# ZhuorenLi/MPC_motion_planning

Measured on AMD Instinct MI355X. Metric: mpc_solves_per_sec, higher is better.
Workload: dtype f64

## Files before the change

mpc_motion_planning_amd/csrc/mpcb_api.hip:

```cpp
#include <hip/hip_runtime.h>
#include <rccl/rccl.h>
#include <dlfcn.h>

#include <cmath>
#include <cstdarg>
#include <cstdio>
#include <cstring>
#include <limits>
#include <map>
#include <mutex>
#include <string>
#include <thread>
#include <vector>

#include "mpcb_kernel_dyn.h"
#include "mpcb_dispatch.h"
#include "mpcb_eval.h"
#include "mpcb_multi.h"
#include "mpcb_plant.h"

#ifndef MPCB_WAVES_PER_SIMD
#define MPCB_WAVES_PER_SIMD 1
#endif

namespace {

constexpr double INF = std::numeric_limits<double>::infinity();
thread_local std::string g_create_error;

template <int NOBS, bool GEN, bool RK4> constexpr bool mpcb_kin_fuses = mpcbd::fuses(NOBS, GEN, RK4);
template <int NOBS> constexpr bool mpcb_dyn_fuses = mpcbd::fuses(NOBS, false, false);
__host__ __device__ inline bool mpcb_second_kind1(const mpcb_config& c, const void* z0) {
  return c.init_rollout && (c.second_start == 1 || (c.second_start == 3 && !z0));
}
__device__ __forceinline__ bool mpcb_second_attempt_here(const MpcbKArgs& a, int b, int pass) {
  if (pass != MPCB_PASS_FIRST || !mpcb_second_kind1(a.cfg, a.z0) || !a.status) return false;
  __builtin_amdgcn_fence(__ATOMIC_SEQ_CST, "workgroup");
  const int st = __builtin_nontemporal_load(a.status + (size_t)b * a.st_stride);
  return st != MPCB_ST_SOLVED && st != MPCB_ST_ACCEPTABLE && st != MPCB_ST_INFEASIBLE_X0;
}

template <int NOBS, bool GEN, bool RK4> constexpr bool mpcb_kin_restores = mpcbd::restores_here(MPCB_MODEL_KIN, NOBS, GEN, RK4);
__device__ __forceinline__ bool mpcb_resto_here(const MpcbKArgs& a, int b) {
  const MpcbKArgs& al = *wv::late_args(a);
  if (!al.resto_here || !al.status) return false;
  __builtin_amdgcn_fence(__ATOMIC_SEQ_CST, "workgroup");
  return __builtin_nontemporal_load(al.status + (size_t)b * al.st_stride) == MPCB_ST_NEEDS_RESTO;
}

template <int NOBS, bool GEN = false, bool RK4 = false>
__global__ __launch_bounds__(64, MPCB_WAVES_PER_SIMD) void mpcb_kernel_kin(const MpcbKArgs a) {
  extern __shared__ __attribute__((aligned(16))) double mpcb_lds[];
  if constexpr (mpcb_kin_fuses<NOBS, GEN, RK4>) {
    int pass = a.pass;
#pragma clang loop unroll(disable)
    for (;;) {
      mpcb_solve_kin<NOBS, GEN, false, RK4>(a, (int)blockIdx.x, mpcb_lds, pass);
      if (!mpcb_second_attempt_here(a, (int)blockIdx.x, pass)) break;
      pass = MPCB_PASS_SECOND;
    }
  } else {
    mpcb_solve_kin<NOBS, GEN, false, RK4>(a, (int)blockIdx.x, mpcb_lds, a.pass);
  }
  if constexpr (mpcb_kin_restores<NOBS, GEN, RK4>) {
    if (mpcb_resto_here(a, (int)blockIdx.x)) mpcb_solve_kin<NOBS, GEN, true, RK4>(a, (int)blockIdx.x, mpcb_lds, MPCB_PASS_RESTO);
  }
}

template <int NOBS, bool GEN = false, bool RK4 = false>
__global__ __launch_bounds__(64, 1) void mpcb_kernel_kin_resto(const MpcbKArgs a) {
  extern __shared__ __attribute__((aligned(16))) double mpcb_lds[];
  mpcb_solve_kin<NOBS, GEN, true, RK4>(a, (int)blockIdx.x, mpcb_lds, MPCB_PASS_RESTO);
}

template <int NOBS, bool GEN = false, bool RK4 = false>
__global__ __launch_bounds__(64, MPCB_WAVES_PER_SIMD) void mpcb_track_kin(const MpcbKArgs a) {
  extern __shared__ __attribute__((aligned(16))) double mpcb_lds[];
  if constexpr (mpcb_kin_fuses<NOBS, GEN, RK4>) {
    int pass = a.pass;
#pragma clang loop unroll(disable)
    for (;;) {
      mpcb_solve_kin<NOBS, GEN, false, RK4, true>(a, (int)blockIdx.x, mpcb_lds, pass);
      if (!mpcb_second_attempt_here(a, (int)blockIdx.x, pass)) break;
      pass = MPCB_PASS_SECOND;
    }
  } else {
    mpcb_solve_kin<NOBS, GEN, false, RK4, true>(a, (int)blockIdx.x, mpcb_lds, a.pass);
  }
  if constexpr (mpcb_kin_restores<NOBS, GEN, RK4>) {
    if (mpcb_resto_here(a, (int)blockIdx.x)) mpcb_solve_kin<NOBS, GEN, true, RK4, true>(a, (int)blockIdx.x, mpcb_lds, MPCB_PASS_RESTO);
  }
}

template <int NOBS, bool GEN = false, bool RK4 = false>
__global__ __launch_bounds__(64, 1) void mpcb_track_kin_resto(const MpcbKArgs a) {
  extern __shared__ __attribute__((aligned(16))) double mpcb_lds[];
  mpcb_solve_kin<NOBS, GEN, true, RK4, true>(a, (int)blockIdx.x, mpcb_lds, MPCB_PASS_RESTO);
}

template <int NOBS>
__global__ __launch_bounds__(64, MPCB_WAVES_PER_SIMD) void mpcb_kernel_dyn(const MpcbKArgs a) {
  extern __shared__ __attribute__((aligned(16))) double mpcb_lds[];
  if constexpr (mpcb_dyn_fuses<NOBS>) {
    int pass = a.pass;
#pragma clang loop unroll(disable)
    for (;;) {
      mpcb_solve_dyn<NOBS>(a, (int)blockIdx.x, mpcb_lds, pass);
      if (!mpcb_second_attempt_here(a, (int)blockIdx.x, pass)) break;
      pass = MPCB_PASS_SECOND;
    }
  } else {
    mpcb_solve_dyn<NOBS>(a, (int)blockIdx.x, mpcb_lds, a.pass);
  }
}

template <int NOBS>
__global__ __launch_bounds__(64, 1) void mpcb_kernel_dyn_resto(const MpcbKArgs a) {
  extern __shared__ __attribute__((aligned(16))) double mpcb_lds[];
  mpcb_solve_dyn<NOBS, true>(a, (int)blockIdx.x, mpcb_lds, MPCB_PASS_RESTO);
}

template <int NOBS>
__global__ __launch_bounds__(64, MPCB_WAVES_PER_SIMD) void mpcb_param_kin(const MpcbKArgs a) {
  extern __shared__ __attribute__((aligned(16))) double mpcb_lds[];
  if constexpr (mpcb_kin_fuses<NOBS, false, false>) {
    int pass = a.pass;
#pragma clang loop unroll(disable)
    for (;;) {
      mpcb_solve_kin<NOBS, false, false, false, false, true>(a, (int)blockIdx.x, mpcb_lds, pass);
      if (!mpcb_second_attempt_here(a, (int)blockIdx.x, pass)) break;
      pass = MPCB_PASS_SECOND;
    }
  } else {
    mpcb_solve_kin<NOBS, false, false, false, false, true>(a, (int)blockIdx.x, mpcb_lds, a.pass);
  }
  if constexpr (mpcb_kin_restores<NOBS, false, false>) {
    if (mpcb_resto_here(a, (int)blockIdx.x)) mpcb_solve_kin<NOBS, false, true, false, false, true>(a, (int)blockIdx.x, mpcb_lds, MPCB_PASS_RESTO);
  }
}

template <int NOBS>
__global__ __launch_bounds__(64, 1) void mpcb_param_kin_resto(const MpcbKArgs a) {
  extern __shared__ __attribute__((aligned(16))) double mpcb_lds[];
  mpcb_solve_kin<NOBS, false, true, false, false, true>(a, (int)blockIdx.x, mpcb_lds, MPCB_PASS_RESTO);
}

template <int NOBS>
__global__ __launch_bounds__(64, MPCB_WAVES_PER_SIMD) void mpcb_param_dyn(const MpcbKArgs a) {
  extern __shared__ __attribute__((aligned(16))) double mpcb_lds[];
  if constexpr (mpcb_dyn_fuses<NOBS>) {
    int pass = a.pass;
#pragma clang loop unroll(disable)
    for (;;) {
      mpcb_solve_dyn<NOBS, false, true>(a, (int)blockIdx.x, mpcb_lds, pass);
      if (!mpcb_second_attempt_here(a, (int)blockIdx.x, pass)) break;
      pass = MPCB_PASS_SECOND;
    }
  } else {
    mpcb_solve_dyn<NOBS, false, true>(a, (int)blockIdx.x, mpcb_lds, a.pass);
  }
}

template <int NOBS>
__global__ __launch_bounds__(64, 1) void mpcb_param_dyn_resto(const MpcbKArgs a) {
  extern __shared__ __attribute__((aligned(16))) double mpcb_lds[];
  mpcb_solve_dyn<NOBS, true, true>(a, (int)blockIdx.x, mpcb_lds, MPCB_PASS_RESTO);
}

template <int NX, bool PARAMS>
__global__ __launch_bounds__(64) void mpcb_eval(const MpcbEvalArgs a) {
  extern __shared__ __attribute__((aligned(16))) double mpcb_lds[];
  ::mpcb_eval<NX, PARAMS>(a, (int)blockIdx.x, mpcb_lds);
}

__global__ __launch_bounds__(64) void mpcb_multi_expand(const MpcbMultiArgs a) { mpcbm::expand(a, (int)blockIdx.x); }
__global__ __launch_bounds__(64) void mpcb_multi_select(const MpcbMultiArgs a) { mpcbm::select(a, (int)blockIdx.x); }


template <int NX>
__global__ __launch_bounds__(128) void mpcb_advance(const mpcb_config c0, const mpcb_config* __restrict__ cfgs, int B, int nz,
                                                    const double* __restrict__ z, double* __restrict__ x0, double* __restrict__ z0,
                                                    double* __restrict__ obs, double* __restrict__ x_hist, double* __restrict__ u_hist,
                                                    const int32_t* __restrict__ status, int st_stride, int step, int steps,
                                                    int move_obs, int hold, double T) {
  const int b = blockIdx.x * blockDim.x + threadIdx.x;
  if (b >= B) return;
  const mpcb_config& c = cfgs ? cfgs[b] : c0;
  double* xb = x0 + (size_t)b * NX;
  double u[2];
  mpcbp::commit<NX>(c0.N, hold, status[(size_t)b * st_stride], z + (size_t)b * nz, z0 + (size_t)b * nz, u);
  mpcbp::plant<NX>(c, T, u, move_obs, xb, obs + (size_t)b * c0.n_obs * 6);
  if (u_hist) { u_hist[((size_t)b * steps + step) * 2] = u[0]; u_hist[((size_t)b * steps + step) * 2 + 1] = u[1]; }
  if (x_hist) {
    double* h = x_hist + ((size_t)b * (steps + 1) + step + 1) * NX;
#pragma unroll
    for (int q = 0; q < NX; ++q) h[q] = xb[q];
  }
}

// ... 168 lines not shown
struct mpcb_params {
  mpcb_handle* owner = nullptr;
  int32_t B = 0;
  mpcb_config base;
  mpcb_config* d_cfgs = nullptr;
};

struct mpcb_loop {
  mpcb_handle* owner = nullptr;
  int32_t B = 0, flags = 0;
  int id = 0;
  const mpcb_params* params = nullptr;
  double* d_w = nullptr;
  double* d_z = nullptr;
  double* d_traj = nullptr;
  int32_t* d_st = nullptr;
  int32_t* d_it = nullptr;
  int32_t* d_cnt = nullptr;
};

struct mpcb_handle {
  mpcb_config cfg;
  int device = 0;
  hipStream_t stream = nullptr;
  hipStream_t first_stream = nullptr;
  std::string err;
  int nx = 4, nz = 0, ng = 0;
  void* d_buf = nullptr; size_t d_cap = 0;
  void* d_multi = nullptr; size_t multi_cap = 0;
  static constexpr int EV_RING = 256;
  std::vector<std::pair<hipEvent_t, hipEvent_t>> ev;
  int ev_head = 0, ev_pending = 0;
  int launches = 0; double total_ms = 0, last_ms = 0;
  struct Lane { hipStream_t stream = nullptr; double* d_work = nullptr; int32_t* d_st_own = nullptr; int work_cap = 0; hipEvent_t done = nullptr; bool busy = false; };
  std::vector<Lane> lanes;
  int lane_base = 0;
  int inflight() const { return lanes.empty() ? 1 : (int)lanes.size() - lane_base; }
  int next_lane = 0;
  int last_solve_lane = 0;
  hipEvent_t ev_fork = nullptr;
  std::vector<std::vector<hipEvent_t>> marks;
  std::vector<double> tgrid_host;
  ncclComm_t comm = nullptr; int world = 1, rank = 0;
  std::vector<mpcb_handle*> peers;
  double* d_gather = nullptr; size_t gather_cap = 0;
  double* d_red = nullptr;
  double* d_tgrid = nullptr; double T0 = 0;
  hipEvent_t ev_sync = nullptr;
  size_t gathered_rows = 0;
  int64_t gathered_B = 0;
  std::vector<mpcb_params*> params;
  std::vector<mpcb_loop*> loops;
  int loops_created = 0;
  bool resto_in_launch = true;
  bool lane0_own_stream = true;
  bool skip_empty_pass = true;
};

namespace {

int fail(mpcb_handle* h, int code, const char* fmt, ...) {
  char buf[512];
  va_list ap; va_start(ap, fmt); vsnprintf(buf, sizeof buf, fmt, ap); va_end(ap);
  if (h) h->err = buf; else g_create_error = buf;
  return code;
}
#define HIP_TRY(h, expr)                                                                         \
  do { hipError_t e_ = (expr); if (e_ != hipSuccess) return fail(h, MPCB_E_DEVICE, "%s: %s", #expr, hipGetErrorString(e_)); } while (0)

struct Rccl {
  decltype(&ncclGetUniqueId) GetUniqueId; decltype(&ncclCommInitRank) CommInitRank; decltype(&ncclCommInitAll) CommInitAll;
  decltype(&ncclCommDestroy) CommDestroy; decltype(&ncclAllGather) AllGather; decltype(&ncclAllReduce) AllReduce;
  decltype(&ncclGroupStart) GroupStart; decltype(&ncclGroupEnd) GroupEnd; decltype(&ncclGetErrorString) GetErrorString;
};
std::string g_rccl_error;
const Rccl* rccl() {
  static Rccl R; static int state = 0;
  static std::once_flag once;
  std::call_once(once, [] {
    const char* forced = std::getenv("MPCB_RCCL_LIB");
    void* so = nullptr;
    if (forced && *forced) so = dlopen(forced, RTLD_NOW | RTLD_GLOBAL);
    else {
      so = dlopen("librccl.so.1", RTLD_NOW | RTLD_GLOBAL);
      if (!so) so = dlopen("librccl.so", RTLD_NOW | RTLD_GLOBAL);
      if (!so) so = dlopen("/opt/rocm/lib/librccl.so.1", RTLD_NOW | RTLD_GLOBAL);
    }
    if (!so) { const char* e = dlerror(); g_rccl_error = e ? e : "dlopen failed"; state = -1; return; }
    bool ok = true;
// ... 59 lines not shown

int variant_or_fail(mpcb_handle* h, const mpcb_config& c, bool track, bool params, mpcbd::Variant* v) {
  const mpcbd::Refusal r = mpcbd::variant_of(c, track, params, v);
  return r.code == MPCB_OK ? MPCB_OK : fail(h, r.code, r.fmt, c.n_obs);
}

int harvest_one(mpcb_handle* h) {
  const int i = (h->ev_head - h->ev_pending + 2 * mpcb_handle::EV_RING) % mpcb_handle::EV_RING;
  HIP_TRY(h, hipEventSynchronize(h->ev[i].second));
  float ms = 0;
  HIP_TRY(h, hipEventElapsedTime(&ms, h->ev[i].first, h->ev[i].second));
  h->total_ms += ms; h->last_ms = ms; ++h->launches; --h->ev_pending;
  return MPCB_OK;
}

int collect_timing(mpcb_handle* h) {
  while (h->ev_pending > 0) { int rc = harvest_one(h); if (rc != MPCB_OK) return rc; }
  return MPCB_OK;
}

std::mutex g_lds_mutex;
std::map<std::pair<const void*, int>, size_t> g_lds_limit;

template <class K>
int launch_kernel(mpcb_handle* h, hipStream_t stream, K kernel, const MpcbKArgs& a, size_t lds) {
  if (lds > 48 * 1024) {
    std::lock_guard<std::mutex> lock(g_lds_mutex);
    size_t& cur = g_lds_limit[{(const void*)kernel, h->device}];
    if (lds > cur) {
      HIP_TRY(h, hipFuncSetAttribute((const void*)kernel, hipFuncAttributeMaxDynamicSharedMemorySize, (int)lds));
      cur = lds;
    }
  }
  hipLaunchKernelGGL(kernel, dim3(a.B), dim3(64), lds, stream, a);
  return MPCB_OK;
}

int join_lanes(mpcb_handle* h) {
  for (auto& L : h->lanes) {
    if (L.busy) { HIP_TRY(h, hipStreamWaitEvent(h->stream, L.done, 0)); L.busy = false; }
  }
  return MPCB_OK;
}

int ensure_lanes(mpcb_handle* h, int k) {
  for (auto& L : h->lanes) {
    if (L.d_work) (void)hipFree(L.d_work);
    if (L.d_st_own) (void)hipFree(L.d_st_own);
    if (L.done) (void)hipEventDestroy(L.done);
    if (L.stream && L.stream != h->stream && L.stream != h->first_stream) (void)hipStreamDestroy(L.stream);
  }
  h->lanes.clear();
  if (h->stream != h->first_stream) { (void)hipStreamDestroy(h->stream); h->stream = h->first_stream; }
  h->lane_base = (k > 1 && h->lane0_own_stream) ? 1 : 0;
  h->lanes.resize(1);
  for (int j = h->lane_base ? 0 : 1; j < k; ++j) {
    mpcb_handle::Lane L;
    if (j == 0) L.stream = h->first_stream;
    else HIP_TRY(h, hipStreamCreateWithFlags(&L.stream, hipStreamNonBlocking));
    HIP_TRY(h, hipEventCreateWithFlags(&L.done, hipEventDisableTiming));
    h->lanes.push_back(L);
  }
  if (h->lane_base) HIP_TRY(h, hipStreamCreateWithFlags(&h->stream, hipStreamNonBlocking));
  h->lanes[0].stream = h->stream;
  if (!h->ev_fork) HIP_TRY(h, hipEventCreateWithFlags(&h->ev_fork, hipEventDisableTiming));
  h->next_lane = 0; h->last_solve_lane = 0;
  return MPCB_OK;
}

int lane_follows_handle(mpcb_handle* h, int lane) {
  if (h->lanes.empty()) { int rc = ensure_lanes(h, 1); if (rc != MPCB_OK) return rc; }
  const hipStream_t s = h->lanes[lane].stream;
  if (s == h->stream) return MPCB_OK;
  if (h->lane0_own_stream) {
    const hipError_t q = hipStreamQuery(h->stream);
    if (q == hipSuccess) return MPCB_OK;
    (void)hipGetLastError();
    if (q != hipErrorNotReady) return fail(h, MPCB_E_DEVICE, "hipStreamQuery: %s", hipGetErrorString(q));
  }
  HIP_TRY(h, hipEventRecord(h->ev_fork, h->stream));
  HIP_TRY(h, hipStreamWaitEvent(s, h->ev_fork, 0));
  return MPCB_OK;
}

template <class T> constexpr auto kernel_of(T) {
  constexpr int n = T::nobs;
  constexpr bool g = T::gen, r = T::rk4;
  if constexpr (T::model == MPCB_MODEL_DYN) {
    if constexpr (T::params) { if constexpr (T::resto) return mpcb_param_dyn_resto<n>; else return mpcb_param_dyn<n>; }
    else { if constexpr (T::resto) return mpcb_kernel_dyn_resto<n>; else return mpcb_kernel_dyn<n>; }
  } else if constexpr (T::params) { if constexpr (T::resto) return mpcb_param_kin_resto<n>; else return mpcb_param_kin<n>; }
  else if constexpr (T::track) { if constexpr (T::resto) return mpcb_track_kin_resto<n, g, r>; else return mpcb_track_kin<n, g, r>; }
  else { if constexpr (T::resto) return mpcb_kernel_kin_resto<n, g, r>; else return mpcb_kernel_kin<n, g, r>; }
}

int launch_solve(mpcb_handle* h, const MpcbKArgs& a_in, int lane_id = 0) {
  MpcbKArgs a = a_in;
// ... 9 lines not shown
  { int rc = lane_follows_handle(h, lane_id); if (rc != MPCB_OK) return rc; }
  mpcb_handle::Lane& L = h->lanes[lane_id];
  const hipStream_t stream = L.stream;
  a.work = nullptr;
  if (mpcbd::multi_pass(h->cfg)) {
    if (a.B > L.work_cap) {
      HIP_TRY(h, hipStreamSynchronize(stream));
      if (L.d_work) HIP_TRY(h, hipFree(L.d_work));
      if (L.d_st_own) HIP_TRY(h, hipFree(L.d_st_own));
      L.d_work = nullptr; L.d_st_own = nullptr; L.work_cap = 0;
      HIP_TRY(h, hipMalloc(&L.d_work, (size_t)a.B * mpcbk::WK_SIZE * sizeof(double)));
      HIP_TRY(h, hipMalloc(&L.d_st_own, (size_t)a.B * sizeof(int32_t)));
      L.work_cap = a.B;
    }
    a.work = L.d_work;
    if (!a.status) {
      if (a.st_stride != 1) return fail(h, MPCB_E_INVALID, "a strided iteration history needs a status history");
      a.status = L.d_st_own;
    }
  }
  if (h->ev.empty()) {
    h->ev.resize(mpcb_handle::EV_RING);
    for (auto& p : h->ev) { HIP_TRY(h, hipEventCreate(&p.first)); HIP_TRY(h, hipEventCreate(&p.second)); }
  }
  if (h->ev_pending == mpcb_handle::EV_RING) { int rc = harvest_one(h); if (rc != MPCB_OK) return rc; }
  auto& evp = h->ev[h->ev_head];
  HIP_TRY(h, hipEventRecord(evp.first, stream));
  for (int i = 0; i < plan.n; ++i) {
    a.pass = plan.pass[i];
    const bool resto = a.pass == MPCB_PASS_RESTO;
    const int force = h->resto_in_launch ? -1 : 0;
    if (h->skip_empty_pass && mpcbd::pass_is_empty(v, h->cfg.N, plan, i, force)) continue;
    a.resto_here = mpcbd::resto_in_launch(v, h->cfg.N, plan, i, force) ? 1 : 0;
    int rc = mpcbd::visit(v, resto, [&](auto inst) { return launch_kernel(h, stream, kernel_of(inst), a, lds[resto || a.resto_here]); });
    if (rc != MPCB_OK) return rc;
    HIP_TRY(h, hipGetLastError());
  }
  HIP_TRY(h, hipEventRecord(evp.second, stream));
  h->ev_head = (h->ev_head + 1) % mpcb_handle::EV_RING; ++h->ev_pending;
  if (stream != h->stream) { HIP_TRY(h, hipEventRecord(L.done, stream)); L.busy = true; }
  return MPCB_OK;
}

int check_track(mpcb_handle* h) {
  mpcbd::Variant v;
  { int rc = variant_or_fail(h, h->cfg, true, false, &v); if (rc != MPCB_OK) return rc; }
  if (!h->peers.empty()) return fail(h, MPCB_E_UNSUPPORTED, "per-stage reference tracking does not run on a device group (mpcb_set_devices)");
  return MPCB_OK;
}

int ensure_scratch(mpcb_handle* h, size_t bytes) {
  if (bytes <= h->d_cap) return MPCB_OK;
  if (h->d_buf) { HIP_TRY(h, hipFree(h->d_buf)); h->d_buf = nullptr; h->d_cap = 0; }
  HIP_TRY(h, hipMalloc(&h->d_buf, bytes));
  h->d_cap = bytes;
  return MPCB_OK;
}

struct Carve {
  char* base; size_t off = 0;
  template <class T> T* take(size_t n) { off = (off + 255) & ~size_t(255); T* p = base ? (T*)(base + off) : nullptr; off += n * sizeof(T); return p; }
  size_t bytes() const { return off + 256; }
};

struct SolveArgs {
  int32_t B = 0; const double *x0 = nullptr, *xs = nullptr, *obs = nullptr; int32_t obs_kind = MPCB_OBSIN_STATIC; const double* z0 = nullptr;
  double *z = nullptr, *obj = nullptr; int32_t *status = nullptr, *iters = nullptr; double *kkt = nullptr, *lam_g = nullptr, *lam_x = nullptr;
// ... 235 lines not shown
  return MPCB_OK;
}

int mpcb_dims(const mpcb_config* c, int32_t* nx, int32_t* nz, int32_t* ng) {
  if (!c) return MPCB_E_INVALID;
  const int n = nx_of(*c);
  if (nx) *nx = n;
  if (nz) *nz = 2 * c->N + n * (c->N + 1);
  if (ng) *ng = n * (c->N + 1) + n_rate(*c) * (c->N - 1) + c->n_obs * (c->obs_terminal ? c->N + 1 : c->N);
  return MPCB_OK;
}

int mpcb_device_count(void) {
  int n = 0;
  if (hipGetDeviceCount(&n) != hipSuccess) return 0;
  return n;
}

int mpcb_create(const mpcb_config* cfg, int32_t device, mpcb_handle** out) {
  if (!out) return fail(nullptr, MPCB_E_INVALID, "out is NULL");
  *out = nullptr;
  int rc = check_cfg(nullptr, cfg);
  if (rc != MPCB_OK) return rc;
  int ndev = 0;
  hipError_t e = hipGetDeviceCount(&ndev);
  if (e != hipSuccess || ndev <= 0) return fail(nullptr, MPCB_E_DEVICE, "no HIP device available (%s); libmpcbatch has no CPU path", e != hipSuccess ? hipGetErrorString(e) : "0 devices");
  if (device < 0 || device >= ndev) return fail(nullptr, MPCB_E_INVALID, "device %d outside 0..%d", device, ndev - 1);
  mpcb_handle* h = new mpcb_handle();
  h->cfg = *cfg; h->device = device;
  const auto switched_off = [](const char* name) { const char* e = std::getenv(name); return e && e[0] == '0' && e[1] == 0; };
  h->resto_in_launch = !switched_off("MPCB_RESTO_IN_LAUNCH");
  h->lane0_own_stream = !switched_off("MPCB_LANE0_OWN_STREAM");
  h->skip_empty_pass = !switched_off("MPCB_SKIP_EMPTY_PASS");
  int nx, nz, ng; mpcb_dims(cfg, &nx, &nz, &ng);
  h->nx = nx; h->nz = nz; h->ng = ng;
  if (hipSetDevice(device) != hipSuccess || hipStreamCreateWithFlags(&h->stream, hipStreamNonBlocking) != hipSuccess) {
    delete h;
    return fail(nullptr, MPCB_E_DEVICE, "cannot create a stream on device %d", device);
  }
  h->first_stream = h->stream;
  *out = h;
  return MPCB_OK;
}

int mpcb_destroy(mpcb_handle* h) {
  if (!h) return MPCB_OK;
  (void)hipSetDevice(h->device);
  collect_timing(h);
  for (auto& p : h->ev) { (void)hipEventDestroy(p.first); (void)hipEventDestroy(p.second); }
  if (h->d_buf) (void)hipFree(h->d_buf);
  if (h->d_multi) (void)hipFree(h->d_multi);
  for (auto* p : h->params) { if (p->d_cfgs) (void)hipFree(p->d_cfgs); delete p; }
  for (auto* p : h->peers) mpcb_destroy(p);
  if (h->comm) { const Rccl* R = rccl(); if (R) (void)R->CommDestroy(h->comm); }
  if (h->d_gather) (void)hipFree(h->d_gather);
  if (h->d_red) (void)hipFree(h->d_red);
  if (h->ev_sync) (void)hipEventDestroy(h->ev_sync);
  if (h->d_tgrid) (void)hipFree(h->d_tgrid);
  for (auto& L : h->lanes) {
    if (L.stream && L.stream != h->stream) { (void)hipStreamSynchronize(L.stream); (void)hipStreamDestroy(L.stream); }
    if (L.d_work) (void)hipFree(L.d_work);
    if (L.d_st_own) (void)hipFree(L.d_st_own);
    if (L.done) (void)hipEventDestroy(L.done);
  }
  if (h->ev_fork) (void)hipEventDestroy(h->ev_fork);
  for (auto& m : h->marks) for (auto e : m) (void)hipEventDestroy(e);
  if (h->stream) (void)hipStreamSynchronize(h->stream);
  for (auto* L : h->loops) { free_loop_buffers(L); delete L; }
  if (h->stream) (void)hipStreamDestroy(h->stream);
  delete h;
  return MPCB_OK;
}

const char* mpcb_last_error(const mpcb_handle* h) { return h ? h->err.c_str() : g_create_error.c_str(); }

int mpcb_set_bounds(mpcb_handle* h, const double* lbx, const double* ubx, int32_t nz, const double* lbg, const double* ubg, int32_t ng) {
  if (!h || !lbx || !ubx || !lbg || !ubg) return fail(h, MPCB_E_INVALID, "NULL argument");
  mpcb_config c = h->cfg;
  const int N = c.N, nx = h->nx;
  if (nz != h->nz) return fail(h, MPCB_E_BOUNDS, "len(lbx) = %d, the NLP has %d variables", nz, h->nz);
  for (int k = 0; k < N; ++k) for (int i = 0; i < 2; ++i)
    if (lbx[2 * k + i] != lbx[i] || ubx[2 * k + i] != ubx[i]) return fail(h, MPCB_E_BOUNDS, "control box differs at stage %d", k);
  for (int k = 0; k <= N; ++k) for (int i = 0; i < nx; ++i)
    if (lbx[2 * N + nx * k + i] != lbx[2 * N + i] || ubx[2 * N + nx * k + i] != ubx[2 * N + i]) return fail(h, MPCB_E_BOUNDS, "state box differs at node %d", k);
  for (int i = 0; i < 2; ++i) { c.u_lo[i] = lbx[i]; c.u_hi[i] = ubx[i]; }
  for (int i = 0; i < nx; ++i) { c.x_lo[i] = lbx[2 * N + i]; c.x_hi[i] = ubx[2 * N + i]; }
  const int n_obs_rows = c.n_obs * (c.obs_terminal ? N + 1 : N);
  const int n_eq = nx * (N + 1);
  const int rate_rows = ng - n_eq - n_obs_rows;
  if (rate_rows < 0 || (rate_rows != 0 && rate_rows % (N - 1 > 0 ? N - 1 : 1) != 0) || (N > 1 && rate_rows / (N - 1) > 2))
    return fail(h, MPCB_E_BOUNDS, "len(lbg) = %d does not match %d equality + k*(N-1) rate + %d obstacle rows", ng, n_eq, n_obs_rows);
  const int nr = (N > 1) ? rate_rows / (N - 1) : 0;
  std::vector<int> kind(ng, 0);
  int r = 0;
  if (!c.rate_interleaved) {
// ... 1095 lines not shown
```

mpc_motion_planning_amd/csrc/mpcb_dispatch.h:

```cpp
#pragma once

#include <cstddef>
#include <utility>

namespace mpcbd {

struct Variant {
  int model, nobs;
  bool gen, rk4, track, params;
};
constexpr bool operator==(const Variant& a, const Variant& b) {
  return a.model == b.model && a.nobs == b.nobs && a.gen == b.gen && a.rk4 == b.rk4 && a.track == b.track && a.params == b.params;
}

constexpr bool shipped(const Variant& v) {
  const int n = v.nobs;
  if (v.track && v.params) return false;
  if (v.model == MPCB_MODEL_DYN) return !v.gen && !v.rk4 && !v.track && (n == 1 || n == 3 || (!v.params && (n == 5 || n == 8)));
  if (v.model != MPCB_MODEL_KIN || (v.gen && v.rk4)) return false;
  if (v.params) return !v.gen && !v.rk4 && (n == 0 || n == 1 || n == 3);
  if (v.gen) return n == 1 || n == 3 || n == 8;
  if (v.rk4) return n == 0 || n == 1 || n == 3;
  return n == 0 || n == 1 || n == 3 || n == 5 || n == 8;
}
// ... 45 lines not shown
  Plan p{0, {0, 0, 0, 0}};
  const bool kind1 = second_kind1(c, start_given);
  p.pass[p.n++] = MPCB_PASS_FIRST;
  if (c.restoration && !kind1) p.pass[p.n++] = MPCB_PASS_RESTO;
  if (second_pass(c)) {
    if (!(kind1 && fused)) p.pass[p.n++] = MPCB_PASS_SECOND;
    if (c.restoration) p.pass[p.n++] = MPCB_PASS_RESTO;
  }
  return p;
}

#ifdef MPCB_NO_RESTO_IN_LAUNCH
constexpr int RESTO_HERE_NOBS_MAX = -1;
#else
constexpr int RESTO_HERE_NOBS_MAX = 1;
#endif
constexpr bool restores_here(int model, int nobs, bool gen, bool rk4) {
  return model == MPCB_MODEL_KIN && nobs <= RESTO_HERE_NOBS_MAX && !gen && !rk4;
}
constexpr bool restores_here(const Variant& v) { return restores_here(v.model, v.nobs, v.gen, v.rk4); }

constexpr int wgs_per_cu(size_t lds) { return lds == 0 || LDS_MAX_BYTES / lds >= 4 ? 4 : (int)(LDS_MAX_BYTES / lds); }

inline bool resto_in_launch(const Variant& v, int N, const Plan& plan, int i, int force = -1) {
  if (force == 0 || !restores_here(v)) return false;
  if (plan.pass[i] == MPCB_PASS_RESTO || i + 1 >= plan.n || plan.pass[i + 1] != MPCB_PASS_RESTO) return false;
  return force == 1 || wgs_per_cu(lds_bytes(v, N, true)) >= wgs_per_cu(lds_bytes(v, N, false));
}

inline bool pass_is_empty(const Variant& v, int N, const Plan& plan, int i, int force = -1) {
  return i > 0 && plan.pass[i] == MPCB_PASS_RESTO && resto_in_launch(v, N, plan, i - 1, force);
}

template <int MODEL, int NOBS, bool GEN, bool RK4, bool TRACK, bool PARAMS, bool RESTO>
struct Inst {
  static constexpr int model = MODEL, nobs = NOBS;
  static constexpr bool gen = GEN, rk4 = RK4, track = TRACK, params = PARAMS, resto = RESTO;
};

namespace detail {
constexpr int CAPS[5] = {0, 1, 3, 5, 8};
constexpr Variant candidate(int I) { return {(I / 5) % 2 ? MPCB_MODEL_DYN : MPCB_MODEL_KIN, CAPS[I % 5], (I / 20) % 2 != 0, (I / 10) % 2 != 0, (I / 40) % 2 != 0, (I / 80) % 2 != 0}; }
constexpr int CANDIDATES = 160;
constexpr int count_shipped() { int n = 0; for (int i = 0; i < CANDIDATES; ++i) n += shipped(candidate(i)) ? 1 : 0; return n; }
static_assert(2 * count_shipped() == 62, "the library ships 62 solve instantiations");

template <bool RESTO, int I, class F>
bool visit_one(const Variant& v, F& f, int& rc) {
  constexpr Variant c = candidate(I);
  if constexpr (shipped(c)) {
    if (v == c) { rc = f(Inst<c.model, c.nobs, c.gen, c.rk4, c.track, c.params, RESTO>{}); return true; }
  }
  return false;
}
template <bool RESTO, class F, int... I>
int visit_all(const Variant& v, F& f, std::integer_sequence<int, I...>) {
  int rc = -1;
  (void)(visit_one<RESTO, I>(v, f, rc) || ...);
  return rc;
}
}

template <bool RESTO, class F>
int visit(const Variant& v, F&& f) { return detail::visit_all<RESTO>(v, f, std::make_integer_sequence<int, detail::CANDIDATES>{}); }
template <class F>
int visit(const Variant& v, bool resto, F&& f) { return resto ? visit<true>(v, f) : visit<false>(v, f); }
// ... 3 lines not shown
```

mpc_motion_planning_amd/csrc/mpcb_kernel.h:

```cpp
#pragma once

#include "../../include/mpcbatch.h"
#include "mpcb_wave.h"

#ifdef MPCB_WAVE_EMU
#include <cmath>
using std::log; using std::fabs; using std::sqrt; using std::pow; using std::fmin; using std::fmax; using std::rint; using std::fma;
using std::isfinite;
#endif

struct MpcbKArgs {
  mpcb_config cfg;
  int32_t B, nz, ng, obs_kind, want_mult, trace_instance;
  int32_t st_stride;
  int32_t pass;
  const double* tgrid;
  double* work;
  const double *x0, *xs, *obs, *z0;
  double *z, *obj, *kkt, *lam_g, *lam_x;
  int32_t *status, *iters;
  double* trace;
  const double* xref;
  const mpcb_config* cfgs;
  int32_t resto_here;
};

#if defined(MPCB_STAMPS) && !defined(MPCB_WAVE_EMU)
#define MPCB_STAMP(var) unsigned long long var = __builtin_amdgcn_s_memtime()
#else
#define MPCB_STAMP(var) unsigned long long var = 0
#endif
#ifndef MPCB_WAVE_EMU
#define MPCB_SCHED_FENCE() __builtin_amdgcn_sched_barrier(0)
#else
#define MPCB_SCHED_FENCE() ((void)0)
#endif

#ifdef MPCB_LATE_TRACE
#define MPCB_TRACE_ARGS(a) wv::late_args(a)
#else
#define MPCB_TRACE_ARGS(a) (&(a))
#endif
#define MPCB_ST_NEEDS_RESTO 7
#define MPCB_PASS_FIRST 0
#define MPCB_PASS_SECOND 1
#define MPCB_PASS_RESTO 2

namespace mpcbk {

template <bool PARAMS> MPCB_DEV const mpcb_config& cfg_late(const MpcbKArgs& a, const int b) {
  if constexpr (PARAMS) return *wv::late_row(wv::late_args(a)->cfgs, b);
  else return wv::late_args(a)->cfg;
}

constexpr int NU = 2;
constexpr int FILTER_MAX = 64;
constexpr double RS_RHO = 1000.0, RS_KAPPA = 0.5, RS_GAP = 10.0, TRIG_ALPHA = 0.05, TRIG_THETA = 0.8;
// ... 1482 lines not shown
```

Measured before the change: 2.290 million.

## Add persistent grid with atomic ticket work-stealing for small-obstacle solve kernels

Launches solve kernels with a grid sized to the number of resident workgroup slots (CUs times workgroups per CU) instead of one block per instance. Each block then pulls further instance indices from a device-wide atomic ticket counter until the batch is exhausted. The last block to retire resets the counter for the next launch. The aim is to cut block scheduling and launch-tail overhead and to balance variable-length solves. The cost is an atomic per instance, a sync between instances, and an extra per-lane ticket buffer.

```diff
diff --git a/mpc_motion_planning_amd/csrc/mpcb_api.hip b/mpc_motion_planning_amd/csrc/mpcb_api.hip
--- a/mpc_motion_planning_amd/csrc/mpcb_api.hip
+++ b/mpc_motion_planning_amd/csrc/mpcb_api.hip
@@ -4,6 +4,7 @@
 
 #include <cmath>
 #include <cstdarg>
+#include <cstdlib>
 #include <cstdio>
 #include <cstring>
 #include <limits>
@@ -15,6 +16,7 @@
 
 #include "mpcb_kernel_dyn.h"
 #include "mpcb_dispatch.h"
+#include "mpcb_grid.h"
 #include "mpcb_eval.h"
 #include "mpcb_multi.h"
 #include "mpcb_plant.h"
@@ -48,29 +50,43 @@
   return __builtin_nontemporal_load(al.status + (size_t)b * al.st_stride) == MPCB_ST_NEEDS_RESTO;
 }
 
+template <bool LOOPS, class F>
+__device__ __forceinline__ void mpcb_grid_loop(const MpcbKArgs& a, F&& one) {
+  if constexpr (!LOOPS) {
+    one((int)blockIdx.x);
+  } else {
+    const auto late = [&a]() __attribute__((always_inline)) { return wv::late_args(a); };
+    mpcbg::for_each_instance(mpcbg::DeviceTicket<decltype(late)>{late}, (int)blockIdx.x, one, []() __attribute__((always_inline)) { wv::sync(); });
+  }
+}
+
 template <int NOBS, bool GEN = false, bool RK4 = false>
 __global__ __launch_bounds__(64, MPCB_WAVES_PER_SIMD) void mpcb_kernel_kin(const MpcbKArgs a) {
   extern __shared__ __attribute__((aligned(16))) double mpcb_lds[];
-  if constexpr (mpcb_kin_fuses<NOBS, GEN, RK4>) {
-    int pass = a.pass;
+  mpcb_grid_loop<mpcbd::loops(NOBS, GEN, RK4)>(a, [&](const int b) __attribute__((always_inline)) {
+    if constexpr (mpcb_kin_fuses<NOBS, GEN, RK4>) {
+      int pass = a.pass;
 #pragma clang loop unroll(disable)
-    for (;;) {
-      mpcb_solve_kin<NOBS, GEN, false, RK4>(a, (int)blockIdx.x, mpcb_lds, pass);
-      if (!mpcb_second_attempt_here(a, (int)blockIdx.x, pass)) break;
-      pass = MPCB_PASS_SECOND;
+      for (;;) {
+        mpcb_solve_kin<NOBS, GEN, false, RK4>(a, b, mpcb_lds, pass);
+        if (!mpcb_second_attempt_here(a, b, pass)) break;
+        pass = MPCB_PASS_SECOND;
+      }
+    } else {
+      mpcb_solve_kin<NOBS, GEN, false, RK4>(a, b, mpcb_lds, a.pass);
     }
-  } else {
-    mpcb_solve_kin<NOBS, GEN, false, RK4>(a, (int)blockIdx.x, mpcb_lds, a.pass);
-  }
-  if constexpr (mpcb_kin_restores<NOBS, GEN, RK4>) {
-    if (mpcb_resto_here(a, (int)blockIdx.x)) mpcb_solve_kin<NOBS, GEN, true, RK4>(a, (int)blockIdx.x, mpcb_lds, MPCB_PASS_RESTO);
-  }
+    if constexpr (mpcb_kin_restores<NOBS, GEN, RK4>) {
+      if (mpcb_resto_here(a, b)) mpcb_solve_kin<NOBS, GEN, true, RK4>(a, b, mpcb_lds, MPCB_PASS_RESTO);
+    }
+  });
 }
 
 template <int NOBS, bool GEN = false, bool RK4 = false>
 __global__ __launch_bounds__(64, 1) void mpcb_kernel_kin_resto(const MpcbKArgs a) {
   extern __shared__ __attribute__((aligned(16))) double mpcb_lds[];
-  mpcb_solve_kin<NOBS, GEN, true, RK4>(a, (int)blockIdx.x, mpcb_lds, MPCB_PASS_RESTO);
+  mpcb_grid_loop<mpcbd::loops(NOBS, GEN, RK4)>(a, [&](const int b) __attribute__((always_inline)) {
+    mpcb_solve_kin<NOBS, GEN, true, RK4>(a, b, mpcb_lds, MPCB_PASS_RESTO);
+  });
 }
 
 template <int NOBS, bool GEN = false, bool RK4 = false>
@@ -101,70 +117,82 @@
 template <int NOBS>
 __global__ __launch_bounds__(64, MPCB_WAVES_PER_SIMD) void mpcb_kernel_dyn(const MpcbKArgs a) {
   extern __shared__ __attribute__((aligned(16))) double mpcb_lds[];
-  if constexpr (mpcb_dyn_fuses<NOBS>) {
-    int pass = a.pass;
+  mpcb_grid_loop<mpcbd::loops(NOBS, false, false)>(a, [&](const int b) __attribute__((always_inline)) {
+    if constexpr (mpcb_dyn_fuses<NOBS>) {
+      int pass = a.pass;
 #pragma clang loop unroll(disable)
-    for (;;) {
-      mpcb_solve_dyn<NOBS>(a, (int)blockIdx.x, mpcb_lds, pass);
-      if (!mpcb_second_attempt_here(a, (int)blockIdx.x, pass)) break;
-      pass = MPCB_PASS_SECOND;
+      for (;;) {
+        mpcb_solve_dyn<NOBS>(a, b, mpcb_lds, pass);
+        if (!mpcb_second_attempt_here(a, b, pass)) break;
+        pass = MPCB_PASS_SECOND;
+      }
+    } else {
+      mpcb_solve_dyn<NOBS>(a, b, mpcb_lds, a.pass);
     }
-  } else {
-    mpcb_solve_dyn<NOBS>(a, (int)blockIdx.x, mpcb_lds, a.pass);
-  }
+  });
 }
 
 template <int NOBS>
 __global__ __launch_bounds__(64, 1) void mpcb_kernel_dyn_resto(const MpcbKArgs a) {
   extern __shared__ __attribute__((aligned(16))) double mpcb_lds[];
-  mpcb_solve_dyn<NOBS, true>(a, (int)blockIdx.x, mpcb_lds, MPCB_PASS_RESTO);
+  mpcb_grid_loop<mpcbd::loops(NOBS, false, false)>(a, [&](const int b) __attribute__((always_inline)) {
+    mpcb_solve_dyn<NOBS, true>(a, b, mpcb_lds, MPCB_PASS_RESTO);
+  });
 }
 
 template <int NOBS>
 __global__ __launch_bounds__(64, MPCB_WAVES_PER_SIMD) void mpcb_param_kin(const MpcbKArgs a) {
   extern __shared__ __attribute__((aligned(16))) double mpcb_lds[];
-  if constexpr (mpcb_kin_fuses<NOBS, false, false>) {
-    int pass = a.pass;
+  mpcb_grid_loop<mpcbd::loops(NOBS, false, false)>(a, [&](const int b) __attribute__((always_inline)) {
+    if constexpr (mpcb_kin_fuses<NOBS, false, false>) {
+      int pass = a.pass;
 #pragma clang loop unroll(disable)
-    for (;;) {
-      mpcb_solve_kin<NOBS, false, false, false, false, true>(a, (int)blockIdx.x, mpcb_lds, pass);
-      if (!mpcb_second_attempt_here(a, (int)blockIdx.x, pass)) break;
-      pass = MPCB_PASS_SECOND;
+      for (;;) {
+        mpcb_solve_kin<NOBS, false, false, false, false, true>(a, b, mpcb_lds, pass);
+        if (!mpcb_second_attempt_here(a, b, pass)) break;
+        pass = MPCB_PASS_SECOND;
+      }
+    } else {
+      mpcb_solve_kin<NOBS, false, false, false, false, true>(a, b, mpcb_lds, a.pass);
     }
-  } else {
-    mpcb_solve_kin<NOBS, false, false, false, false, true>(a, (int)blockIdx.x, mpcb_lds, a.pass);
-  }
-  if constexpr (mpcb_kin_restores<NOBS, false, false>) {
-    if (mpcb_resto_here(a, (int)blockIdx.x)) mpcb_solve_kin<NOBS, false, true, false, false, true>(a, (int)blockIdx.x, mpcb_lds, MPCB_PASS_RESTO);
-  }
+    if constexpr (mpcb_kin_restores<NOBS, false, false>) {
+      if (mpcb_resto_here(a, b)) mpcb_solve_kin<NOBS, false, true, false, false, true>(a, b, mpcb_lds, MPCB_PASS_RESTO);
+    }
+  });
 }
 
 template <int NOBS>
 __global__ __launch_bounds__(64, 1) void mpcb_param_kin_resto(const MpcbKArgs a) {
   extern __shared__ __attribute__((aligned(16))) double mpcb_lds[];
-  mpcb_solve_kin<NOBS, false, true, false, false, true>(a, (int)blockIdx.x, mpcb_lds, MPCB_PASS_RESTO);
+  mpcb_grid_loop<mpcbd::loops(NOBS, false, false)>(a, [&](const int b) __attribute__((always_inline)) {
+    mpcb_solve_kin<NOBS, false, true, false, false, true>(a, b, mpcb_lds, MPCB_PASS_RESTO);
+  });
 }
 
 template <int NOBS>
 __global__ __launch_bounds__(64, MPCB_WAVES_PER_SIMD) void mpcb_param_dyn(const MpcbKArgs a) {
   extern __shared__ __attribute__((aligned(16))) double mpcb_lds[];
-  if constexpr (mpcb_dyn_fuses<NOBS>) {
-    int pass = a.pass;
+  mpcb_grid_loop<mpcbd::loops(NOBS, false, false)>(a, [&](const int b) __attribute__((always_inline)) {
+    if constexpr (mpcb_dyn_fuses<NOBS>) {
+      int pass = a.pass;
 #pragma clang loop unroll(disable)
-    for (;;) {
-      mpcb_solve_dyn<NOBS, false, true>(a, (int)blockIdx.x, mpcb_lds, pass);
-      if (!mpcb_second_attempt_here(a, (int)blockIdx.x, pass)) break;
-      pass = MPCB_PASS_SECOND;
+      for (;;) {
+        mpcb_solve_dyn<NOBS, false, true>(a, b, mpcb_lds, pass);
+        if (!mpcb_second_attempt_here(a, b, pass)) break;
+        pass = MPCB_PASS_SECOND;
+      }
+    } else {
+      mpcb_solve_dyn<NOBS, false, true>(a, b, mpcb_lds, a.pass);
     }
-  } else {
-    mpcb_solve_dyn<NOBS, false, true>(a, (int)blockIdx.x, mpcb_lds, a.pass);
-  }
+  });
 }
 
 template <int NOBS>
 __global__ __launch_bounds__(64, 1) void mpcb_param_dyn_resto(const MpcbKArgs a) {
   extern __shared__ __attribute__((aligned(16))) double mpcb_lds[];
-  mpcb_solve_dyn<NOBS, true, true>(a, (int)blockIdx.x, mpcb_lds, MPCB_PASS_RESTO);
+  mpcb_grid_loop<mpcbd::loops(NOBS, false, false)>(a, [&](const int b) __attribute__((always_inline)) {
+    mpcb_solve_dyn<NOBS, true, true>(a, b, mpcb_lds, MPCB_PASS_RESTO);
+  });
 }
 
 template <int NX, bool PARAMS>
@@ -399,7 +427,8 @@
   std::vector<std::pair<hipEvent_t, hipEvent_t>> ev;
   int ev_head = 0, ev_pending = 0;
   int launches = 0; double total_ms = 0, last_ms = 0;
-  struct Lane { hipStream_t stream = nullptr; double* d_work = nullptr; int32_t* d_st_own = nullptr; int work_cap = 0; hipEvent_t done = nullptr; bool busy = false; };
+  struct Lane { hipStream_t stream = nullptr; double* d_work = nullptr; int32_t* d_st_own = nullptr; int work_cap = 0; hipEvent_t done = nullptr; bool busy = false;
+                int32_t* d_ticket = nullptr; };
   std::vector<Lane> lanes;
   int lane_base = 0;
   int inflight() const { return lanes.empty() ? 1 : (int)lanes.size() - lane_base; }
@@ -422,6 +451,9 @@
   bool resto_in_launch = true;
   bool lane0_own_stream = true;
   bool skip_empty_pass = true;
+  int persistent_grid = -1;
+  int grid_cap = 0;
+  int cus = 0;
 };
 
 namespace {
@@ -547,7 +579,7 @@
       cur = lds;
     }
   }
-  hipLaunchKernelGGL(kernel, dim3(a.B), dim3(64), lds, stream, a);
+  hipLaunchKernelGGL(kernel, dim3(a.grid), dim3(64), lds, stream, a);
   return MPCB_OK;
 }
 
@@ -562,6 +594,7 @@
   for (auto& L : h->lanes) {
     if (L.d_work) (void)hipFree(L.d_work);
     if (L.d_st_own) (void)hipFree(L.d_st_own);
+    if (L.d_ticket) (void)hipFree(L.d_ticket);
     if (L.done) (void)hipEventDestroy(L.done);
     if (L.stream && L.stream != h->stream && L.stream != h->first_stream) (void)hipStreamDestroy(L.stream);
   }
@@ -578,6 +611,10 @@
   }
   if (h->lane_base) HIP_TRY(h, hipStreamCreateWithFlags(&h->stream, hipStreamNonBlocking));
   h->lanes[0].stream = h->stream;
+  for (auto& L : h->lanes) {
+    HIP_TRY(h, hipMalloc(&L.d_ticket, mpcbg::TICKET_WORDS * sizeof(int32_t)));
+    HIP_TRY(h, hipMemsetAsync(L.d_ticket, 0, mpcbg::TICKET_WORDS * sizeof(int32_t), L.stream));
+  }
   if (!h->ev_fork) HIP_TRY(h, hipEventCreateWithFlags(&h->ev_fork, hipEventDisableTiming));
   h->next_lane = 0; h->last_solve_lane = 0;
   return MPCB_OK;
@@ -653,7 +690,14 @@
     const int force = h->resto_in_launch ? -1 : 0;
     if (h->skip_empty_pass && mpcbd::pass_is_empty(v, h->cfg.N, plan, i, force)) continue;
     a.resto_here = mpcbd::resto_in_launch(v, h->cfg.N, plan, i, force) ? 1 : 0;
-    int rc = mpcbd::visit(v, resto, [&](auto inst) { return launch_kernel(h, stream, kernel_of(inst), a, lds[resto || a.resto_here]); });
+    const size_t lds_i = lds[resto || a.resto_here];
+    const int slots = mpcbd::slots_of(h->cus, lds_i);
+    a.grid = mpcbd::loops(v) && mpcbd::grid_pays(a.B, slots, h->inflight(), h->persistent_grid) ? mpcbd::grid_size(a.B, slots, h->grid_cap) : a.B;
+    a.ticket = nullptr;
+    if (mpcbd::needs_ticket(a.B, a.grid)) {
+      a.ticket = L.d_ticket;
+    }
+    int rc = mpcbd::visit(v, resto, [&](auto inst) { return launch_kernel(h, stream, kernel_of(inst), a, lds_i); });
     if (rc != MPCB_OK) return rc;
     HIP_TRY(h, hipGetLastError());
   }
@@ -955,9 +999,13 @@
   h->resto_in_launch = !switched_off("MPCB_RESTO_IN_LAUNCH");
   h->lane0_own_stream = !switched_off("MPCB_LANE0_OWN_STREAM");
   h->skip_empty_pass = !switched_off("MPCB_SKIP_EMPTY_PASS");
+  if (const char* e = std::getenv("MPCB_PERSISTENT_GRID")) h->persistent_grid = (e[0] == '0' && e[1] == 0) ? 0 : (e[0] == '1' && e[1] == 0) ? 1 : -1;
+  if (const char* cap = std::getenv("MPCB_GRID_CAP")) h->grid_cap = std::atoi(cap) > 0 ? std::atoi(cap) : 0;
+  if (h->grid_cap > 0 && h->persistent_grid < 0) h->persistent_grid = 1;
   int nx, nz, ng; mpcb_dims(cfg, &nx, &nz, &ng);
   h->nx = nx; h->nz = nz; h->ng = ng;
-  if (hipSetDevice(device) != hipSuccess || hipStreamCreateWithFlags(&h->stream, hipStreamNonBlocking) != hipSuccess) {
+  if (hipSetDevice(device) != hipSuccess || hipDeviceGetAttribute(&h->cus, hipDeviceAttributeMultiprocessorCount, device) != hipSuccess ||
+      hipStreamCreateWithFlags(&h->stream, hipStreamNonBlocking) != hipSuccess) {
     delete h;
     return fail(nullptr, MPCB_E_DEVICE, "cannot create a stream on device %d", device);
   }
@@ -984,6 +1032,7 @@
     if (L.stream && L.stream != h->stream) { (void)hipStreamSynchronize(L.stream); (void)hipStreamDestroy(L.stream); }
     if (L.d_work) (void)hipFree(L.d_work);
     if (L.d_st_own) (void)hipFree(L.d_st_own);
+    if (L.d_ticket) (void)hipFree(L.d_ticket);
     if (L.done) (void)hipEventDestroy(L.done);
   }
   if (h->ev_fork) (void)hipEventDestroy(h->ev_fork);
diff --git a/mpc_motion_planning_amd/csrc/mpcb_dispatch.h b/mpc_motion_planning_amd/csrc/mpcb_dispatch.h
--- a/mpc_motion_planning_amd/csrc/mpcb_dispatch.h
+++ b/mpc_motion_planning_amd/csrc/mpcb_dispatch.h
@@ -101,6 +101,31 @@
   return i > 0 && plan.pass[i] == MPCB_PASS_RESTO && resto_in_launch(v, N, plan, i - 1, force);
 }
 
+#ifndef MPCB_GRID_FACTOR
+#define MPCB_GRID_FACTOR 1
+#endif
+constexpr int GRID_FACTOR = MPCB_GRID_FACTOR;
+constexpr int slots_of(int cus, size_t lds) { return cus * wgs_per_cu(lds); }
+constexpr int grid_size(int B, int slots, int cap) {
+  int g = B;
+  if (slots > 0 && B > slots) { const long long f = (long long)slots * GRID_FACTOR; g = f < B ? (int)f : B; }
+  if (cap > 0 && g > cap) g = cap;
+  return g;
+}
+constexpr int PERSIST_MIN_TRIPS = 8;
+constexpr bool grid_pays(int B, int slots, int lanes, int force = -1) {
+  if (force >= 0) return force != 0;
+  return lanes == 1 || (long long)B >= (long long)PERSIST_MIN_TRIPS * slots;
+}
+constexpr bool needs_ticket(int B, int grid) { return grid < B; }
+#ifdef MPCB_NO_PERSISTENT_GRID
+constexpr int PERSIST_NOBS_MAX = -1;
+#else
+constexpr int PERSIST_NOBS_MAX = 3;
+#endif
+constexpr bool loops(int nobs, bool gen, bool rk4) { return nobs <= PERSIST_NOBS_MAX && !gen && !rk4; }
+constexpr bool loops(const Variant& v) { return !v.track && loops(v.nobs, v.gen, v.rk4); }
+
 template <int MODEL, int NOBS, bool GEN, bool RK4, bool TRACK, bool PARAMS, bool RESTO>
 struct Inst {
   static constexpr int model = MODEL, nobs = NOBS;
diff --git a/mpc_motion_planning_amd/csrc/mpcb_grid.h b/mpc_motion_planning_amd/csrc/mpcb_grid.h
--- /dev/null
+++ b/mpc_motion_planning_amd/csrc/mpcb_grid.h
@@ -0,0 +1,67 @@
+#pragma once
+
+#if defined(__HIPCC__) && !defined(MPCB_WAVE_EMU)
+#include <hip/hip_runtime.h>
+#define MPCB_GRID_FN __device__ __forceinline__
+#else
+#include <atomic>
+#define MPCB_GRID_FN inline
+#endif
+
+namespace mpcbg {
+
+constexpr int TICKET_WORDS = 2;
+
+#if defined(__HIPCC__) && !defined(MPCB_WAVE_EMU)
+template <class Late>
+struct DeviceTicket {
+  using gptr = __attribute__((address_space(1))) int*;
+  Late late;
+  MPCB_GRID_FN bool armed() const { return late()->ticket != nullptr; }
+  MPCB_GRID_FN int grid() const { return late()->grid; }
+  MPCB_GRID_FN int B() const { return late()->B; }
+  MPCB_GRID_FN int draw() const {
+    int t = 0;
+    if (threadIdx.x == 0) t = __hip_atomic_fetch_add((gptr)late()->ticket, 1, __ATOMIC_RELAXED, __HIP_MEMORY_SCOPE_AGENT);
+    return __builtin_amdgcn_readfirstlane(t);
+  }
+  MPCB_GRID_FN void retire() const {
+    if (threadIdx.x == 0) {
+      const gptr w = (gptr)late()->ticket;
+      const int d = __hip_atomic_fetch_add(w + 1, 1, __ATOMIC_ACQ_REL, __HIP_MEMORY_SCOPE_AGENT);
+      if (d == grid() - 1) {
+        __hip_atomic_store(w, 0, __ATOMIC_RELAXED, __HIP_MEMORY_SCOPE_AGENT);
+        __hip_atomic_store(w + 1, 0, __ATOMIC_RELAXED, __HIP_MEMORY_SCOPE_AGENT);
+      }
+    }
+  }
+};
+#else
+struct HostTicket {
+  std::atomic<int>* w; int grid_, B_;
+  bool armed() const { return w != nullptr; }
+  int grid() const { return grid_; }
+  int B() const { return B_; }
+  int draw() const { return w[0].fetch_add(1, std::memory_order_relaxed); }
+  void retire() const {
+    const int d = w[1].fetch_add(1, std::memory_order_acq_rel);
+    if (d == grid_ - 1) { w[0].store(0, std::memory_order_relaxed); w[1].store(0, std::memory_order_relaxed); }
+  }
+};
+#endif
+
+template <class Ticket, class Solve, class Between>
+MPCB_GRID_FN void for_each_instance(const Ticket& ticket, const int g, Solve&& solve, Between&& between) {
+#if defined(__clang__)
+#pragma clang loop unroll(disable)
+#endif
+  for (int b = g; b < ticket.B();) {
+    solve(b);
+    if (!ticket.armed()) return;
+    between();
+    b = ticket.grid() + ticket.draw();
+  }
+  if (ticket.armed()) ticket.retire();
+}
+
+}
diff --git a/mpc_motion_planning_amd/csrc/mpcb_kernel.h b/mpc_motion_planning_amd/csrc/mpcb_kernel.h
--- a/mpc_motion_planning_amd/csrc/mpcb_kernel.h
+++ b/mpc_motion_planning_amd/csrc/mpcb_kernel.h
@@ -23,6 +23,8 @@
   const double* xref;
   const mpcb_config* cfgs;
   int32_t resto_here;
+  int32_t grid;
+  int32_t* ticket;
 };
 
 #if defined(MPCB_STAMPS) && !defined(MPCB_WAVE_EMU)
```

New measurement: 2.292 million, median of 6. No clear change (+0.1%).
